# pyani-plus/pyani-plus

Hardware: AMD Instinct MI355X
Metric: pairwise genome comparisons/sec (N x N ANI matrix) (higher is better)
Workload: dtype u64

## Files before the change

pyani_plus_amd/csrc/kmer_hash.hip:

```cpp
#include <cstdlib>
#include <type_traits>

#include "pa_internal.h"
#include "murmur_dev.h"

namespace {

using namespace pa_dev;

constexpr int kThreads = 256;
constexpr uint32_t kStageCap = 1024;

constexpr int pow2_floor(int k) { int c = 1; while (2 * c <= k) c *= 2; return c; }

__device__ __forceinline__ uint32_t find_genome(const uint32_t *__restrict__ genome_blk, uint32_t n, uint32_t blk) {
  uint32_t lo = 0, hi = n;
  while (hi - lo > 1) {
    uint32_t mid = (lo + hi) >> 1;
    if (genome_blk[mid] <= blk) lo = mid; else hi = mid;
  }
  return lo;
}

__device__ __forceinline__ void region_append(uint64_t *__restrict__ regions, const uint64_t *__restrict__ region_off,
                                              uint32_t *__restrict__ cursor, uint32_t *__restrict__ overflow,
                                              uint32_t g, uint64_t h) {
  const uint64_t slot = atomicAdd(&cursor[g], 1u);
  if (slot < region_off[g + 1] - region_off[g]) regions[region_off[g] + slot] = h; else *overflow = 1u;
}

template <int K, bool LUT>
__global__ __launch_bounds__(kThreads) void kmer_hash_kernel(
    const uint4 *__restrict__ packed, const uint2 *__restrict__ mask, const uint64_t *__restrict__ dirty, uint32_t n_blocks64,
    const uint32_t *__restrict__ genome_blk, uint32_t n_genomes, uint64_t max_hash,
    uint64_t *__restrict__ cand_hash, uint32_t *__restrict__ cand_genome, uint64_t cap,
    unsigned long long *__restrict__ count, const uint64_t *__restrict__ region_off, uint32_t *__restrict__ cursor,
    uint32_t *__restrict__ overflow, uint32_t blk0) {
  static_assert(K >= 1 && K <= 32, "a k-mer is one 64-bit register pair");
  __shared__ uint64_t s_hash[kStageCap];
  __shared__ uint32_t s_blk[kStageCap];
  __shared__ uint32_t s_n;
  __shared__ unsigned long long s_base;
  constexpr int kWords = (K + 7) / 8;
  __shared__ uint64_t s_lo[LUT ? kWords : 1][256];
  __shared__ uint32_t s_hi[LUT ? kWords : 1][256];

  const uint32_t tid = threadIdx.x;
  const uint32_t max_hi = (uint32_t)(max_hash >> 32);
  const bool take_all = max_hi == 0xffffffffu;
  const uint32_t screen_hi = max_hi + 1u;
  if (tid == 0) s_n = 0;
  if constexpr (LUT) {
#pragma unroll
    for (int j = 0; j < kWords; ++j) {
      const uint64_t cj = (j & 1) ? kC2 : kC1;
      s_lo[j][tid] = (uint64_t)ascii_group(tid, K - 8 * j) * cj;
      s_hi[j][tid] = (uint32_t)((uint64_t)ascii_group(tid, K - 8 * j - 4) * cj);
    }
  }
  __syncthreads();

  const uint32_t t = blk0 + blockIdx.x * kThreads + tid;
  if (t < n_blocks64) {
    const uint4 cur = packed[t];
    uint2 pw = make_uint2(0u, 0u);
    if (t > 0) pw = reinterpret_cast<const uint2 *>(packed)[2 * (uint64_t)t - 1];
    uint32_t d1 = 0u, d2 = 0u;
    const uint32_t wave_blk = __builtin_amdgcn_readfirstlane(t & ~63u);
    const uint64_t dirty_word = dirty[wave_blk >> 6];
    if ((dirty_word >> (t & 63u)) & 1ull) {
      const uint2 m = mask[t];
      uint32_t d0 = t > 0 ? mask[t - 1].y : 0xffffffffu;
      d1 = m.x;
      d2 = m.y;
      int c = 1;
#pragma unroll
      for (; 2 * c <= K; c *= 2) {
        d2 |= alignbit(d2, d1, 32 - c);
        d1 |= alignbit(d1, d0, 32 - c);
        d0 |= d0 << c;
      }
      constexpr int cc = pow2_floor(K);
      constexpr int r = K - cc;
      if constexpr (r > 0) {
        d2 |= alignbit(d2, d1, 32 - r);
        d1 |= alignbit(d1, d0, 32 - r);
      }
    }
    const uint32_t bad[2] = {d1, d2};
    if ((d1 & d2) != 0xffffffffu) {
      constexpr uint64_t kMask = (K == 32) ? ~0ULL : ((1ULL << (2 * K)) - 1);
      constexpr uint32_t kMaskHi = (uint32_t)(kMask >> 32);
      uint32_t fw[8] = {pw.x, pw.y, cur.x, cur.y, cur.z, cur.w, 0u, 0u};
      uint32_t rw[6];
#pragma unroll
      for (int j = 0; j < 6; ++j) {
        const uint32_t x = __builtin_bitreverse32(fw[5 - j]);
        rw[j] = ~(((x >> 1) & 0x55555555u) | ((x & 0x55555555u) << 1));
      }
      auto columns = [&](auto base_tag, int i_begin, int i_end) {
        constexpr int kBase = decltype(base_tag)::value;
#pragma unroll 1
        for (int i = i_begin; i < i_end; ++i) {
          constexpr int kOff = 33 - K;
          const uint32_t fo = 2u * (uint32_t)((i + kOff) & 15), ro = 30u - 2u * (uint32_t)i;
          uint32_t A[5], B[5];
#pragma unroll
          for (int j = 0; j < 5; ++j) {
            A[j] = alignbit(fw[kBase + j + 1], fw[kBase + j], fo);
            B[j] = alignbit(rw[j + 1], rw[j], ro);
          }
#pragma unroll
          for (int wi = 0; wi < 4; ++wi) {
            const uint32_t f_lo = A[wi], f_hi = A[wi + 1], r_lo = B[3 - wi], r_hi = B[4 - wi];
          const uint64_t f_lsb = u64_of(f_lo, f_hi) & kMask, r_lsb = u64_of(r_lo, r_hi) & kMask;
          const uint64_t fwd = __builtin_amdgcn_uicmpl(f_lsb, r_lsb, 37 );
          uint32_t clo, chi;
          asm("s_nop 1\n\tv_cndmask_b32_e64 %0, %1, %2, %3" : "=v"(clo) : "v"((uint32_t)r_lsb), "v"((uint32_t)f_lsb), "s"(fwd));
          asm("v_cndmask_b32_e64 %0, %1, %2, %3" : "=v"(chi) : "v"((uint32_t)(r_lsb >> 32)), "v"((uint32_t)(f_lsb >> 32)), "s"(fwd), "v"(clo));
          uint64_t P[4] = {0, 0, 0, 0};
#pragma unroll
          for (int j = 0; j < kWords; ++j) {
            const uint32_t src = j < 2 ? clo : chi;
            const uint32_t glo = (src >> (16 * (j & 1))) & 0xffu, ghi = (src >> (16 * (j & 1) + 8)) & 0xffu;
            if constexpr (LUT) {
              const uint64_t lo = s_lo[j][glo];
              const uint32_t hi = (uint32_t)(lo >> 32) + s_hi[j][ghi];
              P[j] = u64_of((uint32_t)lo, hi);
            } else {
              const uint64_t word = u64_of(ascii_group(glo, K - 8 * j), ascii_group(ghi, K - 8 * j - 4));
              P[j] = word * ((j & 1) ? kC2 : kC1);
            }
          }
          (void)kMaskHi;
          uint64_t U, V;
          murmur3_pre_last_mul<K>(P, U, V);
          if (take_all || last_mul_high_sum_plus1(U, V) <= screen_hi) {
            const uint64_t X = U * kF2, Y = V * kF2;
            const uint64_t h = (X ^ (X >> 33)) + (Y ^ (Y >> 33));
            if (h > max_hash || ((bad[wi >> 1] >> (16 * (wi & 1) + i)) & 1u)) continue;
            const uint32_t slot = atomicAdd(&s_n, 1u);
            if (slot < kStageCap) {
              s_hash[slot] = h;
              s_blk[slot] = t;
            } else if (region_off) {
              region_append(cand_hash, region_off, cursor, overflow, find_genome(genome_blk, n_genomes, t), h);
            } else {
              const unsigned long long g = atomicAdd(count, 1ULL);
              if (g < cap) {
                cand_hash[g] = h;
                cand_genome[g] = find_genome(genome_blk, n_genomes, t);
              }
            }
          }
          }
        }
      };
      constexpr int kOff0 = 33 - K, kSplit = (kOff0 & 15) ? 16 - (kOff0 & 15) : 16;
      columns(std::integral_constant<int, (kOff0 >> 4)>{}, 0, kSplit);
      if constexpr (kSplit < 16) columns(std::integral_constant<int, (kOff0 >> 4) + 1>{}, kSplit, 16);
    }
  }
  __syncthreads();
  const uint32_t n = min(s_n, kStageCap);
  if (n == 0) return;
  if (region_off) {
    const uint32_t b0 = blk0 + blockIdx.x * kThreads;
    const uint32_t b1 = min(b0 + (uint32_t)kThreads, n_blocks64) - 1u;
    const uint32_t g0 = find_genome(genome_blk, n_genomes, b0);
    if (genome_blk[g0 + 1] > b1) {
      if (tid == 0) s_base = atomicAdd(&cursor[g0], n);
      __syncthreads();
      const uint64_t room = region_off[g0 + 1] - region_off[g0];
      uint64_t *__restrict__ dst = cand_hash + region_off[g0];
      for (uint32_t i = tid; i < n; i += kThreads) {
        const uint64_t slot = s_base + i;
        if (slot < room) dst[slot] = s_hash[i]; else *overflow = 1u;
      }
    } else {
      for (uint32_t i = tid; i < n; i += kThreads)
        region_append(cand_hash, region_off, cursor, overflow, find_genome(genome_blk, n_genomes, s_blk[i]), s_hash[i]);
    }
    return;
  }
  if (tid == 0) s_base = atomicAdd(count, (unsigned long long)n);
  __syncthreads();
  const unsigned long long base = s_base;
  for (uint32_t i = tid; i < n; i += kThreads) {
    const unsigned long long g = base + i;
    if (g < cap) {
      cand_hash[g] = s_hash[i];
      cand_genome[g] = find_genome(genome_blk, n_genomes, s_blk[i]);
    }
  }
}

template <int K, bool LUT>
int launch_variant(pa_ctx *c, const uint32_t *d_packed, const uint32_t *d_mask, const uint64_t *d_dirty, uint64_t n_blocks64,
           const uint32_t *d_genome_blk, uint32_t n_genomes, uint64_t max_hash, uint64_t *d_cand_hash,
           uint32_t *d_cand_genome, uint64_t cap, uint64_t *d_count, const uint64_t *d_region_off, uint32_t *d_cursor,
           uint32_t *d_overflow, uint64_t blk0, hipStream_t stream) {
  const uint32_t grid = ceil_div_u64(n_blocks64 - blk0, kThreads);
  hipLaunchKernelGGL((kmer_hash_kernel<K, LUT>), dim3(grid), dim3(kThreads), 0, stream ? stream : c->stream,
                     reinterpret_cast<const uint4 *>(d_packed), reinterpret_cast<const uint2 *>(d_mask), d_dirty,
                     (uint32_t)n_blocks64, d_genome_blk, n_genomes, max_hash, d_cand_hash, d_cand_genome, cap,
                     reinterpret_cast<unsigned long long *>(d_count), d_region_off, d_cursor, d_overflow, (uint32_t)blk0);
  PA_HIP(hipGetLastError());
  return PA_OK;
}

template <int K>
int launch(pa_ctx *c, const uint32_t *d_packed, const uint32_t *d_mask, const uint64_t *d_dirty, uint64_t n_blocks64,
           const uint32_t *d_genome_blk, uint32_t n_genomes, uint64_t max_hash, uint64_t *d_cand_hash,
           uint32_t *d_cand_genome, uint64_t cap, uint64_t *d_count, const uint64_t *d_region_off, uint32_t *d_cursor,
           uint32_t *d_overflow, uint64_t blk0, hipStream_t stream) {
  static const bool arithmetic = [] {
    const char *v = PA_TOOL_ENV("PA_KMER_VARIANT");
    return v && v[0] == '0';
  }();
  if constexpr (K == 31)
    if (arithmetic)
      return launch_variant<K, false>(c, d_packed, d_mask, d_dirty, n_blocks64, d_genome_blk, n_genomes, max_hash, d_cand_hash,
                                    d_cand_genome, cap, d_count, d_region_off, d_cursor, d_overflow, blk0, stream);
  return launch_variant<K, true>(c, d_packed, d_mask, d_dirty, n_blocks64, d_genome_blk, n_genomes, max_hash, d_cand_hash,
                                 d_cand_genome, cap, d_count, d_region_off, d_cursor, d_overflow, blk0, stream);
}

template <int K>
__global__ __launch_bounds__(kThreads) void kmer_hash_wide_kernel(
    const uint4 *__restrict__ packed, const uint2 *__restrict__ mask, const uint64_t *__restrict__ dirty, uint32_t n_blocks64,
    const uint32_t *__restrict__ genome_blk, uint32_t n_genomes, uint64_t max_hash,
    uint64_t *__restrict__ cand_hash, uint32_t *__restrict__ cand_genome, uint64_t cap,
    unsigned long long *__restrict__ count, const uint64_t *__restrict__ region_off, uint32_t *__restrict__ cursor,
    uint32_t *__restrict__ overflow, uint32_t blk0) {
  static_assert(K >= 33 && K <= 64, "k-mers of 65 to 128 bits");
  __shared__ uint64_t s_hash[kStageCap];
  __shared__ uint32_t s_blk[kStageCap];
  __shared__ uint32_t s_n;
  __shared__ unsigned long long s_base;
  constexpr int kWords = (K + 7) / 8;
  __shared__ uint64_t s_lo[kWords][256];
  __shared__ uint32_t s_hi[kWords][256];
  const uint32_t tid = threadIdx.x;
  const uint32_t max_hi = (uint32_t)(max_hash >> 32);
  const bool take_all = max_hi == 0xffffffffu;
  const uint32_t screen_hi = max_hi + 1u;
  if (tid == 0) s_n = 0;
#pragma unroll
  for (int j = 0; j < kWords; ++j) {
    const uint64_t cj = (j & 1) ? kC2 : kC1;
    s_lo[j][tid] = (uint64_t)ascii_group(tid, K - 8 * j) * cj;
    s_hi[j][tid] = (uint32_t)((uint64_t)ascii_group(tid, K - 8 * j - 4) * cj);
  }
  __syncthreads();

  const uint32_t t = blk0 + blockIdx.x * kThreads + tid;
  if (t < n_blocks64) {
    const uint4 cur = packed[t];
    const uint4 prev = t > 0 ? packed[t - 1] : make_uint4(0u, 0u, 0u, 0u);
    uint32_t d2 = 0u, d3 = 0u;
    const uint32_t wave_blk = __builtin_amdgcn_readfirstlane(t & ~63u);
    const uint64_t dirty_word = dirty[wave_blk >> 6];
    const uint64_t before = wave_blk ? dirty[(wave_blk >> 6) - 1] >> 63 : 1ull;
    const uint64_t dirty_or_prev = dirty_word | (dirty_word << 1) | before;
    if ((dirty_or_prev >> (t & 63u)) & 1ull) {
      const uint2 m = mask[t];
      uint32_t d0 = 0xffffffffu, d1 = 0xffffffffu;
      if (t > 0) { const uint2 mp = mask[t - 1]; d0 = mp.x; d1 = mp.y; }
      d2 = m.x;
      d3 = m.y;
#pragma unroll
      for (int c = 1; c <= 16; c *= 2) {
        d3 |= alignbit(d3, d2, 32 - c);
        d2 |= alignbit(d2, d1, 32 - c);
        d1 |= alignbit(d1, d0, 32 - c);
        d0 |= d0 << c;
      }
      if constexpr (K == 64) {
        d3 |= d2; d2 |= d1; d1 |= d0;
      } else {
        constexpr int r = K - 32;
        d3 |= alignbit(d3, d2, 32 - r);
        d2 |= alignbit(d2, d1, 32 - r);
        d1 |= alignbit(d1, d0, 32 - r);
      }
    }
    const uint32_t bad[2] = {d2, d3};
    if ((d2 & d3) != 0xffffffffu) {
      constexpr uint32_t kMask2 = (2 * K - 64 >= 32) ? 0xffffffffu : ((1u << (2 * K - 64)) - 1u);
      constexpr uint32_t kMask3 = (2 * K - 96 >= 32) ? 0xffffffffu : (2 * K - 96 <= 0 ? 0u : ((1u << ((2 * K - 96) & 31)) - 1u));
      const uint32_t fw[10] = {prev.x, prev.y, prev.z, prev.w, cur.x, cur.y, cur.z, cur.w, 0u, 0u};
      uint32_t rw[10];
#pragma unroll
      for (int j = 0; j < 10; ++j) {
        const uint32_t x = __builtin_bitreverse32(fw[9 - j]);
        rw[j] = ~(((x >> 1) & 0x55555555u) | ((x & 0x55555555u) << 1));
      }
      auto columns = [&](auto base_tag, int i_begin, int i_end) {
        constexpr int kBase = decltype(base_tag)::value;
#pragma unroll 1
        for (int i = i_begin; i < i_end; ++i) {
          constexpr int kOff = 65 - K;
          const uint32_t fo = 2u * (uint32_t)((i + kOff) & 15), ro = 30u - 2u * (uint32_t)i;
          uint32_t A[7], B[7];
#pragma unroll
          for (int j = 0; j < 7; ++j) {
            A[j] = alignbit(fw[kBase + j + 1], fw[kBase + j], fo);
            B[j] = alignbit(rw[j + 3], rw[j + 2], ro);
          }
#pragma unroll
          for (int wi = 0; wi < 4; ++wi) {
            const uint32_t f0 = A[wi], f1 = A[wi + 1], f2 = A[wi + 2] & kMask2, f3 = A[wi + 3] & kMask3;
            const uint32_t r0 = B[3 - wi], r1 = B[4 - wi], r2 = B[5 - wi] & kMask2, r3 = B[6 - wi] & kMask3;
            const uint64_t lt_hi = __builtin_amdgcn_uicmpl(u64_of(f2, f3), u64_of(r2, r3), 36 );
            const uint64_t eq_hi = __builtin_amdgcn_uicmpl(u64_of(f2, f3), u64_of(r2, r3), 32 );
            const uint64_t le_lo = __builtin_amdgcn_uicmpl(u64_of(f0, f1), u64_of(r0, r1), 37 );
            const uint64_t fwd = lt_hi | (eq_hi & le_lo);
            uint32_t c0, c1, c2, c3;
            asm("s_nop 1\n\tv_cndmask_b32_e64 %0, %1, %2, %3" : "=v"(c0) : "v"(r0), "v"(f0), "s"(fwd));
            asm("v_cndmask_b32_e64 %0, %1, %2, %3" : "=v"(c1) : "v"(r1), "v"(f1), "s"(fwd), "v"(c0));
            asm("v_cndmask_b32_e64 %0, %1, %2, %3" : "=v"(c2) : "v"(r2), "v"(f2), "s"(fwd), "v"(c1));
            asm("v_cndmask_b32_e64 %0, %1, %2, %3" : "=v"(c3) : "v"(r3), "v"(f3), "s"(fwd), "v"(c2));
            const uint32_t cw[4] = {c0, c1, c2, c3};
            uint64_t P[8] = {0, 0, 0, 0, 0, 0, 0, 0};
#pragma unroll
            for (int j = 0; j < kWords; ++j) {
              const uint32_t src = cw[j >> 1];
              const uint32_t glo = (src >> (16 * (j & 1))) & 0xffu, ghi = (src >> (16 * (j & 1) + 8)) & 0xffu;
              const uint64_t lo = s_lo[j][glo];
              P[j] = u64_of((uint32_t)lo, (uint32_t)(lo >> 32) + s_hi[j][ghi]);
            }
            uint64_t U, V;
            murmur3_pre_last_mul<K>(P, U, V);
            if (take_all || last_mul_high_sum_plus1(U, V) <= screen_hi) {
              const uint64_t X = U * kF2, Y = V * kF2;
              const uint64_t h = (X ^ (X >> 33)) + (Y ^ (Y >> 33));
              if (h > max_hash || ((bad[wi >> 1] >> (16 * (wi & 1) + i)) & 1u)) continue;
              const uint32_t slot = atomicAdd(&s_n, 1u);
              if (slot < kStageCap) {
                s_hash[slot] = h;
                s_blk[slot] = t;
              } else if (region_off) {
                region_append(cand_hash, region_off, cursor, overflow, find_genome(genome_blk, n_genomes, t), h);
              } else {
                const unsigned long long g = atomicAdd(count, 1ULL);
                if (g < cap) {
                  cand_hash[g] = h;
                  cand_genome[g] = find_genome(genome_blk, n_genomes, t);
                }
              }
            }
          }
        }
      };
      constexpr int kOff0 = 65 - K, kSplit = (kOff0 & 15) ? 16 - (kOff0 & 15) : 16;
      columns(std::integral_constant<int, (kOff0 >> 4)>{}, 0, kSplit);
      if constexpr (kSplit < 16) columns(std::integral_constant<int, (kOff0 >> 4) + 1>{}, kSplit, 16);
    }
  }
  __syncthreads();
  const uint32_t n = min(s_n, kStageCap);
  if (n == 0) return;
  if (region_off) {
    const uint32_t b0 = blk0 + blockIdx.x * kThreads;
    const uint32_t b1 = min(b0 + (uint32_t)kThreads, n_blocks64) - 1u;
    const uint32_t g0 = find_genome(genome_blk, n_genomes, b0);
    if (genome_blk[g0 + 1] > b1) {
      if (tid == 0) s_base = atomicAdd(&cursor[g0], n);
      __syncthreads();
      const uint64_t room = region_off[g0 + 1] - region_off[g0];
      uint64_t *__restrict__ dst = cand_hash + region_off[g0];
      for (uint32_t i = tid; i < n; i += kThreads) {
        const uint64_t slot = s_base + i;
        if (slot < room) dst[slot] = s_hash[i]; else *overflow = 1u;
      }
    } else {
      for (uint32_t i = tid; i < n; i += kThreads)
        region_append(cand_hash, region_off, cursor, overflow, find_genome(genome_blk, n_genomes, s_blk[i]), s_hash[i]);
    }
    return;
  }
  if (tid == 0) s_base = atomicAdd(count, (unsigned long long)n);
  __syncthreads();
  const unsigned long long base = s_base;
  for (uint32_t i = tid; i < n; i += kThreads) {
    const unsigned long long g = base + i;
    if (g < cap) {
      cand_hash[g] = s_hash[i];
      cand_genome[g] = find_genome(genome_blk, n_genomes, s_blk[i]);
    }
  }
}

__device__ __forceinline__ uint32_t rev_groups32(uint32_t x) {
  x = __builtin_bitreverse32(x);
  return ((x >> 1) & 0x55555555u) | ((x & 0x55555555u) << 1);
}

__device__ __forceinline__ void murmur3_pre_last_mul_rt(const uint64_t (&P)[8], uint32_t k, uint64_t &U, uint64_t &V) {
  uint64_t h1 = 42, h2 = 42;
  const uint32_t nblocks = k >> 4, tail = k & 15u;
#pragma unroll
  for (uint32_t i = 0; i < 4; ++i) {
    if (i >= nblocks) break;
    h1 ^= rotl64(P[2 * i], 31) * kC2;
    h1 = rotl64(h1, 27) + h2;
    h1 = times5_plus(h1, 0x52dce729ULL);
    h2 ^= rotl64(P[2 * i + 1], 33) * kC1;
    h2 = rotl64(h2, 31) + h1;
    h2 = times5_plus(h2, 0x38495ab5ULL);
  }
  uint64_t t1 = 0, t2 = 0;
#pragma unroll
  for (uint32_t i = 0; i < 4; ++i)
    if (i == nblocks) { t1 = P[2 * i]; t2 = P[2 * i + 1]; }
  if (tail > 8) h2 ^= rotl64(t2, 33) * kC1;
  if (tail > 0) h1 ^= rotl64(t1, 31) * kC2;
  h1 ^= (uint64_t)k;
  h2 ^= (uint64_t)k;
  h1 += h2;
  h2 += h1;
  h1 ^= h1 >> 33; h1 *= kF1; h1 ^= h1 >> 33;
  h2 ^= h2 >> 33; h2 *= kF1; h2 ^= h2 >> 33;
  U = h1;
  V = h2;
}

constexpr int kLongIter = 32;
__global__ __launch_bounds__(kThreads) void kmer_hash_long_kernel(
    const uint32_t *__restrict__ packed, const uint32_t *__restrict__ mask, uint64_t pos0, uint64_t pos1, uint32_t k,
    const uint32_t *__restrict__ genome_blk, uint32_t n_genomes, uint64_t max_hash, uint64_t *__restrict__ cand_hash,
    uint32_t *__restrict__ cand_genome, uint64_t cap, unsigned long long *__restrict__ count,
    const uint64_t *__restrict__ region_off, uint32_t *__restrict__ cursor, uint32_t *__restrict__ overflow) {
  __shared__ uint64_t s_lo[8][256];
  __shared__ uint32_t s_hi[8][256];
  const uint32_t tid = threadIdx.x;
  const uint32_t n_words = (k + 7u) >> 3;
  for (uint32_t j = 0; j < n_words; ++j) {
    const uint64_t cj = (j & 1u) ? kC2 : kC1;
    s_lo[j][tid] = (uint64_t)ascii_group(tid, (int)k - 8 * (int)j) * cj;
    s_hi[j][tid] = (uint32_t)((uint64_t)ascii_group(tid, (int)k - 8 * (int)j - 4) * cj);
  }
  __syncthreads();
  const uint64_t wg_first = pos0 + ((uint64_t)blockIdx.y * gridDim.x + blockIdx.x) * (uint64_t)(kThreads * kLongIter);
#pragma unroll 1
  for (int it = 0; it < kLongIter; ++it) {
  const uint64_t e = wg_first + (uint64_t)it * kThreads + tid;
  if (e >= pos1 || e + 1 < k) continue;
  const uint64_t a = e + 1 - k;
  {
    const uint64_t m0 = a >> 5, m_last = e >> 5;
    const uint32_t sm = (uint32_t)(a & 31u);
    const uint32_t w0 = mask[m0], w1 = m0 + 1 <= m_last ? mask[m0 + 1] : 0u, w2 = m0 + 2 <= m_last ? mask[m0 + 2] : 0u;
    const uint32_t b0 = alignbit(w1, w0, sm), b1 = alignbit(w2, w1, sm);
    const uint32_t top = k == 64 ? 0xffffffffu : ((1u << (k - 32u)) - 1u);
    if (b0 | (b1 & top)) continue;
  }
  uint32_t F[4], R[4];
  {
    const uint64_t p0 = a >> 4, p_last = e >> 4;
    const uint32_t sp = 2u * (uint32_t)(a & 15u);
    uint32_t w[5];
#pragma unroll
    for (int i = 0; i < 5; ++i) w[i] = p0 + i <= p_last ? packed[p0 + i] : 0u;
#pragma unroll
    for (int i = 0; i < 4; ++i) F[i] = alignbit(w[i + 1], w[i], sp);
    const uint32_t used = 2u * k - 64u;
    if (used < 32u) { F[2] &= (1u << used) - 1u; F[3] = 0u; }
    else if (used < 64u) F[3] &= (1u << (used - 32u)) - 1u;
    const uint32_t C[6] = {~rev_groups32(F[3]), ~rev_groups32(F[2]), ~rev_groups32(F[1]), ~rev_groups32(F[0]), 0u, 0u};
    const uint32_t s = 128u - 2u * k, ws = s >> 5, bs = s & 31u;
#pragma unroll
    for (int i = 0; i < 4; ++i) R[i] = ws ? alignbit(C[i + 2], C[i + 1], bs) : alignbit(C[i + 1], C[i], bs);
    if (used < 32u) { R[2] &= (1u << used) - 1u; R[3] = 0u; }
    else if (used < 64u) R[3] &= (1u << (used - 32u)) - 1u;
  }
  const uint64_t f_hi = u64_of(F[2], F[3]), f_lo = u64_of(F[0], F[1]), r_hi = u64_of(R[2], R[3]), r_lo = u64_of(R[0], R[1]);
  const bool fwd = f_hi < r_hi || (f_hi == r_hi && f_lo <= r_lo);
  uint32_t c[4];
#pragma unroll
  for (int i = 0; i < 4; ++i) c[i] = fwd ? F[i] : R[i];
  uint64_t P[8] = {0, 0, 0, 0, 0, 0, 0, 0};
#pragma unroll
  for (uint32_t j = 0; j < 8; ++j) {
    if (j >= n_words) break;
    const uint32_t src = c[j >> 1], glo = (src >> (16u * (j & 1u))) & 0xffu, ghi = (src >> (16u * (j & 1u) + 8u)) & 0xffu;
    const uint64_t lo = s_lo[j][glo];
    P[j] = u64_of((uint32_t)lo, (uint32_t)(lo >> 32) + s_hi[j][ghi]);
  }
  uint64_t U, V;
  murmur3_pre_last_mul_rt(P, k, U, V);
  const uint32_t max_hi = (uint32_t)(max_hash >> 32);
  if (max_hi != 0xffffffffu && last_mul_high_sum_plus1(U, V) > max_hi + 1u) continue;
  const uint64_t X = U * kF2, Y = V * kF2;
  const uint64_t h = (X ^ (X >> 33)) + (Y ^ (Y >> 33));
  if (h > max_hash) continue;
  const uint32_t blk = (uint32_t)(e >> 6);
  const uint32_t g = find_genome(genome_blk, n_genomes, blk);
  if (region_off) {
    region_append(cand_hash, region_off, cursor, overflow, g, h);
  } else {
    const unsigned long long slot = atomicAdd(count, 1ULL);
    if (slot < cap) {
      cand_hash[slot] = h;
      cand_genome[slot] = g;
    }
  }
  }
}

}

int pa_launch_kmer_hash(pa_ctx *c, const uint32_t *d_packed, const uint32_t *d_mask, const uint64_t *d_dirty, uint64_t n_blocks64,
                        const uint32_t *d_genome_blk, uint32_t n_genomes, uint32_t k, uint64_t max_hash,
                        uint64_t *d_cand_hash, uint32_t *d_cand_genome, uint64_t cap, uint64_t *d_count,
                        const uint64_t *d_region_off, uint32_t *d_cursor, uint32_t *d_overflow, uint64_t blk0,
                        hipStream_t stream) {
  PA_REQUIRE(n_blocks64 < (1ULL << 32), "arena too large: %llu blocks of 64 bases", (unsigned long long)n_blocks64);
  if (n_blocks64 <= blk0) return PA_OK;
  const char *long_form = PA_TOOL_ENV("PA_KMER_LONG");
  const bool long_plain = long_form && long_form[0] == 'p';
  if (k > 32 && k <= 64 && !long_plain) {
    PA_REQUIRE((blk0 & 63u) == 0, "k-mer hash launch must start at a multiple of 64 blocks, not %llu", (unsigned long long)blk0);
    const uint32_t grid = ceil_div_u64(n_blocks64 - blk0, kThreads);
#define PA_WIDE_CASE(KK)                                                                                                   \
  case KK:                                                                                                                 \
    hipLaunchKernelGGL((kmer_hash_wide_kernel<KK>), dim3(grid), dim3(kThreads), 0, stream ? stream : c->stream,            \
                       reinterpret_cast<const uint4 *>(d_packed), reinterpret_cast<const uint2 *>(d_mask), d_dirty,        \
                       (uint32_t)n_blocks64, d_genome_blk, n_genomes, max_hash, d_cand_hash, d_cand_genome, cap,           \
                       reinterpret_cast<unsigned long long *>(d_count), d_region_off, d_cursor, d_overflow, (uint32_t)blk0); \
    break;
    switch (k) {
      PA_WIDE_CASE(33) PA_WIDE_CASE(34) PA_WIDE_CASE(35) PA_WIDE_CASE(36) PA_WIDE_CASE(37) PA_WIDE_CASE(38) PA_WIDE_CASE(39)
      PA_WIDE_CASE(40) PA_WIDE_CASE(41) PA_WIDE_CASE(42) PA_WIDE_CASE(43) PA_WIDE_CASE(44) PA_WIDE_CASE(45) PA_WIDE_CASE(46)
      PA_WIDE_CASE(47) PA_WIDE_CASE(48) PA_WIDE_CASE(49) PA_WIDE_CASE(50) PA_WIDE_CASE(51) PA_WIDE_CASE(52) PA_WIDE_CASE(53)
      PA_WIDE_CASE(54) PA_WIDE_CASE(55) PA_WIDE_CASE(56) PA_WIDE_CASE(57) PA_WIDE_CASE(58) PA_WIDE_CASE(59) PA_WIDE_CASE(60)
      PA_WIDE_CASE(61) PA_WIDE_CASE(62) PA_WIDE_CASE(63) PA_WIDE_CASE(64)
      default: break;
    }
#undef PA_WIDE_CASE
    PA_HIP(hipGetLastError());
    return PA_OK;
  }
  if (k > 32 && k <= 64) {
    const uint64_t pos0 = blk0 * 64, pos1 = n_blocks64 * 64;
    const uint64_t per_wg = (uint64_t)kThreads * kLongIter;
    const uint64_t n_wg = (pos1 - pos0 + per_wg - 1) / per_wg;
    const uint32_t gx = (uint32_t)std::min<uint64_t>(n_wg, 1u << 20), gy = (uint32_t)((n_wg + gx - 1) / gx);
    PA_REQUIRE(gy <= 65535u, "arena too large for one launch of the long k-mer kernel: %llu positions", (unsigned long long)(pos1 - pos0));
    hipLaunchKernelGGL(kmer_hash_long_kernel, dim3(gx, gy), dim3(kThreads), 0,
                       stream ? stream : c->stream, d_packed, d_mask, pos0, pos1, k, d_genome_blk, n_genomes, max_hash,
                       d_cand_hash, d_cand_genome, cap, reinterpret_cast<unsigned long long *>(d_count), d_region_off,
                       d_cursor, d_overflow);
    PA_HIP(hipGetLastError());
    return PA_OK;
  }
#define PA_K_CASE(KK) \
  case KK: return launch<KK>(c, d_packed, d_mask, d_dirty, n_blocks64, d_genome_blk, n_genomes, max_hash, d_cand_hash, d_cand_genome, cap, d_count, d_region_off, d_cursor, d_overflow, blk0, stream);
  PA_REQUIRE((blk0 & 63u) == 0, "k-mer hash launch must start at a multiple of 64 blocks, not %llu", (unsigned long long)blk0);
  switch (k) {
    PA_K_CASE(1) PA_K_CASE(2) PA_K_CASE(3) PA_K_CASE(4) PA_K_CASE(5) PA_K_CASE(6) PA_K_CASE(7) PA_K_CASE(8)
    PA_K_CASE(9) PA_K_CASE(10) PA_K_CASE(11) PA_K_CASE(12) PA_K_CASE(13) PA_K_CASE(14) PA_K_CASE(15) PA_K_CASE(16)
    PA_K_CASE(17) PA_K_CASE(18) PA_K_CASE(19) PA_K_CASE(20) PA_K_CASE(21) PA_K_CASE(22) PA_K_CASE(23) PA_K_CASE(24)
    PA_K_CASE(25) PA_K_CASE(26) PA_K_CASE(27) PA_K_CASE(28) PA_K_CASE(29) PA_K_CASE(30) PA_K_CASE(31) PA_K_CASE(32)
    default:
      pa_set_error("k=%u outside [1,64]", k);
      return PA_E_INVALID;
  }
#undef PA_K_CASE
}
```

pyani_plus_amd/csrc/murmur_dev.h:

```cpp
#pragma once

#include <hip/hip_runtime.h>

#include <cstdint>

namespace pa_dev {

__device__ __forceinline__ uint32_t alignbit(uint32_t hi, uint32_t lo, uint32_t sh) {
  return __builtin_amdgcn_alignbit(hi, lo, sh);
}

__device__ __forceinline__ uint32_t ascii4(uint32_t b8) {
  uint32_t u = (b8 | (b8 << 12)) & 0x000F000Fu;
  uint32_t v = (u | (u << 6)) & 0x03030303u;
  return __builtin_amdgcn_perm(0u, 0x54474341u, v);
}

__device__ __forceinline__ uint64_t u64_of(uint32_t lo, uint32_t hi) { return ((uint64_t)hi << 32) | lo; }

__device__ __forceinline__ uint64_t rotl64(uint64_t x, int r) {
  const uint32_t lo = (uint32_t)x, hi = (uint32_t)(x >> 32);
  if (r == 32) return u64_of(hi, lo);
  if (r < 32) return u64_of(alignbit(lo, hi, 32 - r), alignbit(hi, lo, 32 - r));
  return u64_of(alignbit(hi, lo, 64 - r), alignbit(lo, hi, 64 - r));
}

__device__ __forceinline__ uint64_t fmix64(uint64_t k) {
  k ^= k >> 33;
  k *= 0xff51afd7ed558ccdULL;
  k ^= k >> 33;
  k *= 0xc4ceb9fe1a85ec53ULL;
  k ^= k >> 33;
  return k;
}

constexpr uint64_t kC1 = 0x87c37b91114253d5ULL, kC2 = 0x4cf5ad432745937fULL;

__device__ __forceinline__ uint64_t times5_plus(uint64_t h, uint64_t c) {
  uint64_t t;
  asm("v_lshl_add_u64 %0, %1, 2, %1" : "=v"(t) : "v"(h));
  return t + c;
}

constexpr uint64_t kF1 = 0xff51afd7ed558ccdULL, kF2 = 0xc4ceb9fe1a85ec53ULL;

template <int K, int N>
__device__ __forceinline__ void murmur3_pre_last_mul(const uint64_t (&P)[N], uint64_t &U, uint64_t &V) {
  static_assert(N >= (K + 7) / 8, "one first product per 8-byte word of the k-mer");
  uint64_t h1 = 42, h2 = 42;
  constexpr int nblocks = K / 16;
  constexpr int tail = K % 16;
#pragma unroll
  for (int i = 0; i < nblocks; ++i) {
    const uint64_t k1 = rotl64(P[2 * i], 31) * kC2;
    h1 ^= k1;
    if (i == 0) {
      h1 = times5_plus(rotl64(h1, 27), 5ULL * 42ULL + 0x52dce729ULL);
    } else {
      h1 = rotl64(h1, 27) + h2;
      h1 = times5_plus(h1, 0x52dce729ULL);
    }
    const uint64_t k2 = rotl64(P[2 * i + 1], 33) * kC1;
    h2 ^= k2;
    h2 = rotl64(h2, 31) + h1;
    h2 = times5_plus(h2, 0x38495ab5ULL);
  }
  if constexpr (tail > 8) h2 ^= rotl64(P[2 * nblocks + 1], 33) * kC1;
  if constexpr (tail > 0) h1 ^= rotl64(P[2 * nblocks], 31) * kC2;
  h1 ^= (uint64_t)K; h2 ^= (uint64_t)K;
  h1 += h2; h2 += h1;
  h1 ^= h1 >> 33; h1 *= kF1; h1 ^= h1 >> 33;
  h2 ^= h2 >> 33; h2 *= kF1; h2 ^= h2 >> 33;
  U = h1;
  V = h2;
}

__device__ __forceinline__ uint32_t last_mul_high_sum_plus1(uint64_t U, uint64_t V) {
  constexpr uint32_t c0 = (uint32_t)kF2, c1 = (uint32_t)(kF2 >> 32);
  const uint32_t u0 = (uint32_t)U, u1 = (uint32_t)(U >> 32), v0 = (uint32_t)V, v1 = (uint32_t)(V >> 32);
  return (__umulhi(u0, c0) + __umulhi(v0, c0) + 1u) + ((u0 + v0) * c1 + (u1 + v1) * c0);
}

template <int K, int N>
__device__ __forceinline__ uint64_t murmur3_from_products(const uint64_t (&P)[N]) {
  uint64_t U, V;
  murmur3_pre_last_mul<K, N>(P, U, V);
  const uint64_t X = U * kF2, Y = V * kF2;
  return (X ^ (X >> 33)) + (Y ^ (Y >> 33));
}

__device__ __forceinline__ uint32_t ascii_group(uint32_t b8, int nv) {
  const uint32_t a = ascii4(b8);
  return nv >= 4 ? a : (nv <= 0 ? 0u : (a & ((1u << (8 * nv)) - 1u)));
}

}
```

Measured before the change: 79.11 million.

## Precompute the last k-mer word's hashed term in a shared-memory table

When k is not a multiple of 8, the final partial word of the k-mer now indexes a shared table that already holds its fully mixed murmur term (multiply, rotate, multiply). This skips two 64-bit multiplies per k-mer. For larger tables the kernel switches to 1024-thread blocks that each loop over 16 chunks, so the table build is amortised. The pre-filter now sums U and V before a single 64-bit multiply, with a looser bound. Opaque asm barriers are added to steer instruction selection. The candidate-staging code is also factored into a shared sink struct. The trade-offs are more LDS use, lower occupancy, and extra syncs per chunk.

```diff
diff --git a/pyani_plus_amd/csrc/kmer_hash.hip b/pyani_plus_amd/csrc/kmer_hash.hip
--- a/pyani_plus_amd/csrc/kmer_hash.hip
+++ b/pyani_plus_amd/csrc/kmer_hash.hip
@@ -29,38 +29,135 @@
   if (slot < region_off[g + 1] - region_off[g]) regions[region_off[g] + slot] = h; else *overflow = 1u;
 }
 
-template <int K, bool LUT>
-__global__ __launch_bounds__(kThreads) void kmer_hash_kernel(
+struct HashSink {
+  const uint32_t *__restrict__ genome_blk;
+  uint32_t n_genomes;
+  uint64_t *__restrict__ cand_hash;
+  uint32_t *__restrict__ cand_genome;
+  uint64_t cap;
+  unsigned long long *__restrict__ count;
+  const uint64_t *__restrict__ region_off;
+  uint32_t *__restrict__ cursor;
+  uint32_t *__restrict__ overflow;
+
+  __device__ __forceinline__ void keep(uint64_t *s_hash, uint32_t *s_blk, uint32_t *s_n, uint32_t t, uint64_t h) const {
+    const uint32_t slot = atomicAdd(s_n, 1u);
+    if (slot < kStageCap) {
+      s_hash[slot] = h;
+      s_blk[slot] = t;
+    } else if (region_off) {
+      region_append(cand_hash, region_off, cursor, overflow, find_genome(genome_blk, n_genomes, t), h);
+    } else {
+      const unsigned long long g = atomicAdd(count, 1ULL);
+      if (g < cap) {
+        cand_hash[g] = h;
+        cand_genome[g] = find_genome(genome_blk, n_genomes, t);
+      }
+    }
+  }
+
+  template <int kNT>
+  __device__ __forceinline__ void flush(const uint64_t *s_hash, const uint32_t *s_blk, unsigned long long *s_base, uint32_t n,
+                                        uint32_t b0, uint32_t n_blocks64) const {
+    const uint32_t tid = threadIdx.x;
+    if (region_off) {
+      const uint32_t b1 = min(b0 + (uint32_t)kNT, n_blocks64) - 1u;
+      const uint32_t g0 = find_genome(genome_blk, n_genomes, b0);
+      if (genome_blk[g0 + 1] > b1) {
+        if (tid == 0) *s_base = atomicAdd(&cursor[g0], n);
+        __syncthreads();
+        const uint64_t room = region_off[g0 + 1] - region_off[g0];
+        uint64_t *__restrict__ dst = cand_hash + region_off[g0];
+        for (uint32_t i = tid; i < n; i += kNT) {
+          const uint64_t slot = *s_base + i;
+          if (slot < room) dst[slot] = s_hash[i]; else *overflow = 1u;
+        }
+      } else {
+        for (uint32_t i = tid; i < n; i += kNT)
+          region_append(cand_hash, region_off, cursor, overflow, find_genome(genome_blk, n_genomes, s_blk[i]), s_hash[i]);
+      }
+      return;
+    }
+    if (tid == 0) *s_base = atomicAdd(count, (unsigned long long)n);
+    __syncthreads();
+    const unsigned long long base = *s_base;
+    for (uint32_t i = tid; i < n; i += kNT) {
+      const unsigned long long g = base + i;
+      if (g < cap) {
+        cand_hash[g] = s_hash[i];
+        cand_genome[g] = find_genome(genome_blk, n_genomes, s_blk[i]);
+      }
+    }
+  }
+};
+
+enum HashForm { kArithmetic = 0, kTables = 1, kLastWord = 2 };
+
+template <int K, int FORM>
+struct HashShape {
+  static constexpr int kWords = (K + 7) / 8;
+  static constexpr int kLastBases = K - 8 * (kWords - 1);
+  static constexpr bool kLast = FORM == kLastWord;
+  static_assert(!kLast || kLastBases <= 7, "a word of 8 bases is not looked up whole");
+  static constexpr int kSmall = FORM == kArithmetic ? 0 : kWords - (kLast ? 1 : 0);
+  static constexpr uint32_t kBig = kLast ? 1u << (2 * kLastBases) : 0u;
+  static constexpr int kNT = kBig >= 4096u ? 1024 : kThreads;
+  static constexpr int kChunks = kLast ? 16 : 1;
+};
+
+template <int NSMALL, uint32_t NBIG>
+struct HashLds {
+  uint64_t lo[NSMALL ? NSMALL : 1][256];
+  uint32_t hi[NSMALL ? NSMALL : 1][256];
+  uint64_t hash[kStageCap];
+  uint32_t blk[kStageCap];
+  unsigned long long base;
+  uint32_t n;
+  uint64_t big[NBIG ? NBIG : 1];
+};
+
+template <int K>
+__device__ __forceinline__ uint64_t last_word_term(uint32_t w) {
+  constexpr int j = (K + 7) / 8 - 1;
+  const uint64_t word = u64_of(ascii_group(w & 0xffu, K - 8 * j), ascii_group(w >> 8, K - 8 * j - 4));
+  return (j & 1) ? rotl64(word * kC2, 33) * kC1 : rotl64(word * kC1, 31) * kC2;
+}
+
+template <int K, int FORM>
+__global__ __launch_bounds__((HashShape<K, FORM>::kNT)) void kmer_hash_kernel(
     const uint4 *__restrict__ packed, const uint2 *__restrict__ mask, const uint64_t *__restrict__ dirty, uint32_t n_blocks64,
     const uint32_t *__restrict__ genome_blk, uint32_t n_genomes, uint64_t max_hash,
     uint64_t *__restrict__ cand_hash, uint32_t *__restrict__ cand_genome, uint64_t cap,
     unsigned long long *__restrict__ count, const uint64_t *__restrict__ region_off, uint32_t *__restrict__ cursor,
     uint32_t *__restrict__ overflow, uint32_t blk0) {
   static_assert(K >= 1 && K <= 32, "a k-mer is one 64-bit register pair");
-  __shared__ uint64_t s_hash[kStageCap];
-  __shared__ uint32_t s_blk[kStageCap];
-  __shared__ uint32_t s_n;
-  __shared__ unsigned long long s_base;
-  constexpr int kWords = (K + 7) / 8;
-  __shared__ uint64_t s_lo[LUT ? kWords : 1][256];
-  __shared__ uint32_t s_hi[LUT ? kWords : 1][256];
+  using Shape = HashShape<K, FORM>;
+  constexpr int kWords = Shape::kWords, kSmall = Shape::kSmall, kNT = Shape::kNT, kChunks = Shape::kChunks;
+  constexpr bool kLast = Shape::kLast;
+  __shared__ HashLds<kSmall, Shape::kBig> s;
 
   const uint32_t tid = threadIdx.x;
-  const uint32_t max_hi = (uint32_t)(max_hash >> 32);
-  const bool take_all = max_hi == 0xffffffffu;
-  const uint32_t screen_hi = max_hi + 1u;
-  if (tid == 0) s_n = 0;
-  if constexpr (LUT) {
-#pragma unroll
-    for (int j = 0; j < kWords; ++j) {
+  const bool take_all = screen_off(max_hash);
+  const uint32_t screen_hi = screen_bound(max_hash);
+  const HashSink sink{genome_blk, n_genomes, cand_hash, cand_genome, cap, count, region_off, cursor, overflow};
+  if (tid == 0) s.n = 0;
+  if (tid < 256) {
+#pragma unroll
+    for (int j = 0; j < kSmall; ++j) {
       const uint64_t cj = (j & 1) ? kC2 : kC1;
-      s_lo[j][tid] = (uint64_t)ascii_group(tid, K - 8 * j) * cj;
-      s_hi[j][tid] = (uint32_t)((uint64_t)ascii_group(tid, K - 8 * j - 4) * cj);
-    }
-  }
+      s.lo[j][tid] = (uint64_t)ascii_group(tid, K - 8 * j) * cj;
+      s.hi[j][tid] = (uint32_t)((uint64_t)ascii_group(tid, K - 8 * j - 4) * cj);
+    }
+  }
+  if constexpr (kLast)
+    for (uint32_t w = tid; w < Shape::kBig; w += kNT) s.big[w] = last_word_term<K>(w);
   __syncthreads();
 
-  const uint32_t t = blk0 + blockIdx.x * kThreads + tid;
+#pragma unroll 1
+  for (int chunk = 0; chunk < kChunks; ++chunk) {
+  const uint64_t chunk_blk = blk0 + ((uint64_t)blockIdx.x * kChunks + chunk) * kNT;
+  if (chunk_blk >= n_blocks64) break;
+  const uint32_t t = (uint32_t)chunk_blk + tid;
   if (t < n_blocks64) {
     const uint4 cur = packed[t];
     uint2 pw = make_uint2(0u, 0u);
@@ -90,7 +187,6 @@
     const uint32_t bad[2] = {d1, d2};
     if ((d1 & d2) != 0xffffffffu) {
       constexpr uint64_t kMask = (K == 32) ? ~0ULL : ((1ULL << (2 * K)) - 1);
-      constexpr uint32_t kMaskHi = (uint32_t)(kMask >> 32);
       uint32_t fw[8] = {pw.x, pw.y, cur.x, cur.y, cur.z, cur.w, 0u, 0u};
       uint32_t rw[6];
 #pragma unroll
@@ -123,35 +219,24 @@
           for (int j = 0; j < kWords; ++j) {
             const uint32_t src = j < 2 ? clo : chi;
             const uint32_t glo = (src >> (16 * (j & 1))) & 0xffu, ghi = (src >> (16 * (j & 1) + 8)) & 0xffu;
-            if constexpr (LUT) {
-              const uint64_t lo = s_lo[j][glo];
-              const uint32_t hi = (uint32_t)(lo >> 32) + s_hi[j][ghi];
+            if (kLast && j == kWords - 1) {
+              P[j] = s.big[(src >> (16 * (j & 1))) & 0xffffu];
+            } else if (FORM != kArithmetic) {
+              const uint64_t lo = s.lo[j][glo];
+              const uint32_t hi = (uint32_t)(lo >> 32) + s.hi[j][ghi];
               P[j] = u64_of((uint32_t)lo, hi);
             } else {
               const uint64_t word = u64_of(ascii_group(glo, K - 8 * j), ascii_group(ghi, K - 8 * j - 4));
               P[j] = word * ((j & 1) ? kC2 : kC1);
             }
           }
-          (void)kMaskHi;
           uint64_t U, V;
-          murmur3_pre_last_mul<K>(P, U, V);
-          if (take_all || last_mul_high_sum_plus1(U, V) <= screen_hi) {
+          murmur3_pre_last_mul<K, 4, kLast>(P, U, V);
+          if (take_all || last_mul_sum_high_plus1(U, V) <= screen_hi) {
             const uint64_t X = U * kF2, Y = V * kF2;
             const uint64_t h = (X ^ (X >> 33)) + (Y ^ (Y >> 33));
             if (h > max_hash || ((bad[wi >> 1] >> (16 * (wi & 1) + i)) & 1u)) continue;
-            const uint32_t slot = atomicAdd(&s_n, 1u);
-            if (slot < kStageCap) {
-              s_hash[slot] = h;
-              s_blk[slot] = t;
-            } else if (region_off) {
-              region_append(cand_hash, region_off, cursor, overflow, find_genome(genome_blk, n_genomes, t), h);
-            } else {
-              const unsigned long long g = atomicAdd(count, 1ULL);
-              if (g < cap) {
-                cand_hash[g] = h;
-                cand_genome[g] = find_genome(genome_blk, n_genomes, t);
-              }
-            }
+            sink.keep(s.hash, s.blk, &s.n, t, h);
           }
           }
         }
@@ -162,46 +247,24 @@
     }
   }
   __syncthreads();
-  const uint32_t n = min(s_n, kStageCap);
-  if (n == 0) return;
-  if (region_off) {
-    const uint32_t b0 = blk0 + blockIdx.x * kThreads;
-    const uint32_t b1 = min(b0 + (uint32_t)kThreads, n_blocks64) - 1u;
-    const uint32_t g0 = find_genome(genome_blk, n_genomes, b0);
-    if (genome_blk[g0 + 1] > b1) {
-      if (tid == 0) s_base = atomicAdd(&cursor[g0], n);
-      __syncthreads();
-      const uint64_t room = region_off[g0 + 1] - region_off[g0];
-      uint64_t *__restrict__ dst = cand_hash + region_off[g0];
-      for (uint32_t i = tid; i < n; i += kThreads) {
-        const uint64_t slot = s_base + i;
-        if (slot < room) dst[slot] = s_hash[i]; else *overflow = 1u;
-      }
-    } else {
-      for (uint32_t i = tid; i < n; i += kThreads)
-        region_append(cand_hash, region_off, cursor, overflow, find_genome(genome_blk, n_genomes, s_blk[i]), s_hash[i]);
-    }
-    return;
-  }
-  if (tid == 0) s_base = atomicAdd(count, (unsigned long long)n);
-  __syncthreads();
-  const unsigned long long base = s_base;
-  for (uint32_t i = tid; i < n; i += kThreads) {
-    const unsigned long long g = base + i;
-    if (g < cap) {
-      cand_hash[g] = s_hash[i];
-      cand_genome[g] = find_genome(genome_blk, n_genomes, s_blk[i]);
-    }
-  }
-}
-
-template <int K, bool LUT>
+  const uint32_t n = min(s.n, kStageCap);
+  if (n) sink.flush<kNT>(s.hash, s.blk, &s.base, n, (uint32_t)chunk_blk, n_blocks64);
+  if constexpr (kChunks > 1) {
+    __syncthreads();
+    if (tid == 0) s.n = 0;
+    __syncthreads();
+  }
+  }
+}
+
+template <int K, int FORM>
 int launch_variant(pa_ctx *c, const uint32_t *d_packed, const uint32_t *d_mask, const uint64_t *d_dirty, uint64_t n_blocks64,
            const uint32_t *d_genome_blk, uint32_t n_genomes, uint64_t max_hash, uint64_t *d_cand_hash,
            uint32_t *d_cand_genome, uint64_t cap, uint64_t *d_count, const uint64_t *d_region_off, uint32_t *d_cursor,
            uint32_t *d_overflow, uint64_t blk0, hipStream_t stream) {
-  const uint32_t grid = ceil_div_u64(n_blocks64 - blk0, kThreads);
-  hipLaunchKernelGGL((kmer_hash_kernel<K, LUT>), dim3(grid), dim3(kThreads), 0, stream ? stream : c->stream,
+  using Shape = HashShape<K, FORM>;
+  const uint32_t grid = ceil_div_u64(n_blocks64 - blk0, (uint64_t)Shape::kNT * Shape::kChunks);
+  hipLaunchKernelGGL((kmer_hash_kernel<K, FORM>), dim3(grid), dim3(Shape::kNT), 0, stream ? stream : c->stream,
                      reinterpret_cast<const uint4 *>(d_packed), reinterpret_cast<const uint2 *>(d_mask), d_dirty,
                      (uint32_t)n_blocks64, d_genome_blk, n_genomes, max_hash, d_cand_hash, d_cand_genome, cap,
                      reinterpret_cast<unsigned long long *>(d_count), d_region_off, d_cursor, d_overflow, (uint32_t)blk0);
@@ -214,16 +277,23 @@
            const uint32_t *d_genome_blk, uint32_t n_genomes, uint64_t max_hash, uint64_t *d_cand_hash,
            uint32_t *d_cand_genome, uint64_t cap, uint64_t *d_count, const uint64_t *d_region_off, uint32_t *d_cursor,
            uint32_t *d_overflow, uint64_t blk0, hipStream_t stream) {
-  static const bool arithmetic = [] {
+  constexpr bool has_last_table = K % 8 != 0;
+#define PA_HASH_FORM(FORM)                                                                                                  \
+  return launch_variant<K, FORM>(c, d_packed, d_mask, d_dirty, n_blocks64, d_genome_blk, n_genomes, max_hash, d_cand_hash, \
+                                 d_cand_genome, cap, d_count, d_region_off, d_cursor, d_overflow, blk0, stream)
+#ifdef PA_TOOLS
+  if constexpr (K == 31 || K == 21 || K == 16) {
     const char *v = PA_TOOL_ENV("PA_KMER_VARIANT");
-    return v && v[0] == '0';
-  }();
-  if constexpr (K == 31)
-    if (arithmetic)
-      return launch_variant<K, false>(c, d_packed, d_mask, d_dirty, n_blocks64, d_genome_blk, n_genomes, max_hash, d_cand_hash,
-                                    d_cand_genome, cap, d_count, d_region_off, d_cursor, d_overflow, blk0, stream);
-  return launch_variant<K, true>(c, d_packed, d_mask, d_dirty, n_blocks64, d_genome_blk, n_genomes, max_hash, d_cand_hash,
-                                 d_cand_genome, cap, d_count, d_region_off, d_cursor, d_overflow, blk0, stream);
+    if (v && v[0] == '0') PA_HASH_FORM(kArithmetic);
+  }
+  if constexpr (has_last_table) {
+    const char *v = PA_TOOL_ENV("PA_KMER_LAST_WORD");
+    if (v && v[0] == '0') PA_HASH_FORM(kTables);
+  }
+#endif
+  if constexpr (has_last_table) PA_HASH_FORM(kLastWord);
+  else PA_HASH_FORM(kTables);
+#undef PA_HASH_FORM
 }
 
 template <int K>
@@ -238,20 +308,25 @@
   __shared__ uint32_t s_blk[kStageCap];
   __shared__ uint32_t s_n;
   __shared__ unsigned long long s_base;
-  constexpr int kWords = (K + 7) / 8;
-  __shared__ uint64_t s_lo[kWords][256];
-  __shared__ uint32_t s_hi[kWords][256];
+  constexpr int kWords = (K + 7) / 8, kLastBases = K - 8 * (kWords - 1);
+  constexpr bool kLast = kLastBases <= 4;
+  constexpr int kSmall = kWords - (kLast ? 1 : 0);
+  __shared__ uint64_t s_lo[kSmall][256];
+  __shared__ uint32_t s_hi[kSmall][256];
+  __shared__ uint64_t s_big[kLast ? 1 << (2 * kLastBases) : 1];
   const uint32_t tid = threadIdx.x;
-  const uint32_t max_hi = (uint32_t)(max_hash >> 32);
-  const bool take_all = max_hi == 0xffffffffu;
-  const uint32_t screen_hi = max_hi + 1u;
+  const bool take_all = screen_off(max_hash);
+  const uint32_t screen_hi = screen_bound(max_hash);
+  const HashSink sink{genome_blk, n_genomes, cand_hash, cand_genome, cap, count, region_off, cursor, overflow};
   if (tid == 0) s_n = 0;
 #pragma unroll
-  for (int j = 0; j < kWords; ++j) {
+  for (int j = 0; j < kSmall; ++j) {
     const uint64_t cj = (j & 1) ? kC2 : kC1;
     s_lo[j][tid] = (uint64_t)ascii_group(tid, K - 8 * j) * cj;
     s_hi[j][tid] = (uint32_t)((uint64_t)ascii_group(tid, K - 8 * j - 4) * cj);
   }
+  if constexpr (kLast)
+    if (tid < (1u << (2 * kLastBases))) s_big[tid] = last_word_term<K>(tid);
   __syncthreads();
 
   const uint32_t t = blk0 + blockIdx.x * kThreads + tid;
@@ -327,28 +402,20 @@
             for (int j = 0; j < kWords; ++j) {
               const uint32_t src = cw[j >> 1];
               const uint32_t glo = (src >> (16 * (j & 1))) & 0xffu, ghi = (src >> (16 * (j & 1) + 8)) & 0xffu;
-              const uint64_t lo = s_lo[j][glo];
-              P[j] = u64_of((uint32_t)lo, (uint32_t)(lo >> 32) + s_hi[j][ghi]);
+              if (kLast && j == kWords - 1) {
+                P[j] = s_big[glo];
+              } else {
+                const uint64_t lo = s_lo[j < kSmall ? j : 0][glo];
+                P[j] = u64_of((uint32_t)lo, (uint32_t)(lo >> 32) + s_hi[j < kSmall ? j : 0][ghi]);
+              }
             }
             uint64_t U, V;
-            murmur3_pre_last_mul<K>(P, U, V);
-            if (take_all || last_mul_high_sum_plus1(U, V) <= screen_hi) {
+            murmur3_pre_last_mul<K, 8, kLast>(P, U, V);
+            if (take_all || last_mul_sum_high_plus1(U, V) <= screen_hi) {
               const uint64_t X = U * kF2, Y = V * kF2;
               const uint64_t h = (X ^ (X >> 33)) + (Y ^ (Y >> 33));
               if (h > max_hash || ((bad[wi >> 1] >> (16 * (wi & 1) + i)) & 1u)) continue;
-              const uint32_t slot = atomicAdd(&s_n, 1u);
-              if (slot < kStageCap) {
-                s_hash[slot] = h;
-                s_blk[slot] = t;
-              } else if (region_off) {
-                region_append(cand_hash, region_off, cursor, overflow, find_genome(genome_blk, n_genomes, t), h);
-              } else {
-                const unsigned long long g = atomicAdd(count, 1ULL);
-                if (g < cap) {
-                  cand_hash[g] = h;
-                  cand_genome[g] = find_genome(genome_blk, n_genomes, t);
-                }
-              }
+              sink.keep(s_hash, s_blk, &s_n, t, h);
             }
           }
         }
@@ -360,36 +427,7 @@
   }
   __syncthreads();
   const uint32_t n = min(s_n, kStageCap);
-  if (n == 0) return;
-  if (region_off) {
-    const uint32_t b0 = blk0 + blockIdx.x * kThreads;
-    const uint32_t b1 = min(b0 + (uint32_t)kThreads, n_blocks64) - 1u;
-    const uint32_t g0 = find_genome(genome_blk, n_genomes, b0);
-    if (genome_blk[g0 + 1] > b1) {
-      if (tid == 0) s_base = atomicAdd(&cursor[g0], n);
-      __syncthreads();
-      const uint64_t room = region_off[g0 + 1] - region_off[g0];
-      uint64_t *__restrict__ dst = cand_hash + region_off[g0];
-      for (uint32_t i = tid; i < n; i += kThreads) {
-        const uint64_t slot = s_base + i;
-        if (slot < room) dst[slot] = s_hash[i]; else *overflow = 1u;
-      }
-    } else {
-      for (uint32_t i = tid; i < n; i += kThreads)
-        region_append(cand_hash, region_off, cursor, overflow, find_genome(genome_blk, n_genomes, s_blk[i]), s_hash[i]);
-    }
-    return;
-  }
-  if (tid == 0) s_base = atomicAdd(count, (unsigned long long)n);
-  __syncthreads();
-  const unsigned long long base = s_base;
-  for (uint32_t i = tid; i < n; i += kThreads) {
-    const unsigned long long g = base + i;
-    if (g < cap) {
-      cand_hash[g] = s_hash[i];
-      cand_genome[g] = find_genome(genome_blk, n_genomes, s_blk[i]);
-    }
-  }
+  if (n) sink.flush<kThreads>(s_hash, s_blk, &s_base, n, blk0 + blockIdx.x * kThreads, n_blocks64);
 }
 
 __device__ __forceinline__ uint32_t rev_groups32(uint32_t x) {
@@ -490,8 +528,7 @@
   }
   uint64_t U, V;
   murmur3_pre_last_mul_rt(P, k, U, V);
-  const uint32_t max_hi = (uint32_t)(max_hash >> 32);
-  if (max_hi != 0xffffffffu && last_mul_high_sum_plus1(U, V) > max_hi + 1u) continue;
+  if (!screen_off(max_hash) && last_mul_sum_high_plus1(U, V) > screen_bound(max_hash)) continue;
   const uint64_t X = U * kF2, Y = V * kF2;
   const uint64_t h = (X ^ (X >> 33)) + (Y ^ (Y >> 33));
   if (h > max_hash) continue;
diff --git a/pyani_plus_amd/csrc/murmur_dev.h b/pyani_plus_amd/csrc/murmur_dev.h
--- a/pyani_plus_amd/csrc/murmur_dev.h
+++ b/pyani_plus_amd/csrc/murmur_dev.h
@@ -25,6 +25,11 @@
   return u64_of(alignbit(hi, lo, 64 - r), alignbit(lo, hi, 64 - r));
 }
 
+__device__ __forceinline__ uint64_t opaque64(uint64_t x) {
+  asm("" : "+v"(x));
+  return x;
+}
+
 __device__ __forceinline__ uint64_t fmix64(uint64_t k) {
   k ^= k >> 33;
   k *= 0xff51afd7ed558ccdULL;
@@ -44,7 +49,7 @@
 
 constexpr uint64_t kF1 = 0xff51afd7ed558ccdULL, kF2 = 0xc4ceb9fe1a85ec53ULL;
 
-template <int K, int N>
+template <int K, int N, bool kLastReady = false>
 __device__ __forceinline__ void murmur3_pre_last_mul(const uint64_t (&P)[N], uint64_t &U, uint64_t &V) {
   static_assert(N >= (K + 7) / 8, "one first product per 8-byte word of the k-mer");
   uint64_t h1 = 42, h2 = 42;
@@ -57,16 +62,17 @@
     if (i == 0) {
       h1 = times5_plus(rotl64(h1, 27), 5ULL * 42ULL + 0x52dce729ULL);
     } else {
-      h1 = rotl64(h1, 27) + h2;
+      h1 = opaque64(rotl64(h1, 27)) + h2;
       h1 = times5_plus(h1, 0x52dce729ULL);
     }
     const uint64_t k2 = rotl64(P[2 * i + 1], 33) * kC1;
     h2 ^= k2;
-    h2 = rotl64(h2, 31) + h1;
+    h2 = opaque64(rotl64(h2, 31)) + h1;
     h2 = times5_plus(h2, 0x38495ab5ULL);
   }
-  if constexpr (tail > 8) h2 ^= rotl64(P[2 * nblocks + 1], 33) * kC1;
-  if constexpr (tail > 0) h1 ^= rotl64(P[2 * nblocks], 31) * kC2;
+  static_assert(!kLastReady || tail != 0, "a last word of 8 bases has no table");
+  if constexpr (tail > 8) h2 ^= kLastReady ? P[2 * nblocks + 1] : rotl64(P[2 * nblocks + 1], 33) * kC1;
+  if constexpr (tail > 0) h1 ^= (kLastReady && tail <= 8) ? P[2 * nblocks] : rotl64(P[2 * nblocks], 31) * kC2;
   h1 ^= (uint64_t)K; h2 ^= (uint64_t)K;
   h1 += h2; h2 += h1;
   h1 ^= h1 >> 33; h1 *= kF1; h1 ^= h1 >> 33;
@@ -75,11 +81,15 @@
   V = h2;
 }
 
-__device__ __forceinline__ uint32_t last_mul_high_sum_plus1(uint64_t U, uint64_t V) {
+__device__ __forceinline__ uint32_t last_mul_sum_high_plus1(uint64_t U, uint64_t V) {
   constexpr uint32_t c0 = (uint32_t)kF2, c1 = (uint32_t)(kF2 >> 32);
-  const uint32_t u0 = (uint32_t)U, u1 = (uint32_t)(U >> 32), v0 = (uint32_t)V, v1 = (uint32_t)(V >> 32);
-  return (__umulhi(u0, c0) + __umulhi(v0, c0) + 1u) + ((u0 + v0) * c1 + (u1 + v1) * c0);
+  const uint64_t S = U + V;
+  const uint32_t s0 = (uint32_t)S, s1 = (uint32_t)(S >> 32);
+  const uint64_t m = (uint64_t)s0 * c0 + (1ULL << 32);
+  return (uint32_t)(m >> 32) + s0 * c1 + s1 * c0;
 }
+__device__ __forceinline__ bool screen_off(uint64_t max_hash) { return (uint32_t)(max_hash >> 32) >= 0xfffffffeu; }
+__device__ __forceinline__ uint32_t screen_bound(uint64_t max_hash) { return (uint32_t)(max_hash >> 32) + 2u; }
 
 template <int K, int N>
 __device__ __forceinline__ uint64_t murmur3_from_products(const uint64_t (&P)[N]) {
```

After: 73.55 million. 7.0% lower.
